# byu-magicc/VI-EKF

Hardware: AMD Instinct MI355X
Metric: EKF steps/sec (IMU-rate propagate + N_feat updates), batch=1024, N_feat=50 (higher is better)
Workload: dtype f64

## Files before the change

### vi_ekf_amd/csrc/viekf_kernels_resident.hpp

```cpp
#pragma once
#include "viekf_resident_common.hpp"
#include "viekf_resident_prop.hpp"
#include "viekf_resident_worker.hpp"
#include "viekf_resident_service.hpp"

namespace viekf {


template <int T>
__device__ __forceinline__ void res_prologue(const StreamArgs& a, ResShared& S, double* smem, int do_prop,
                                             const double* __restrict__ dt_all, const double* __restrict__ z_all,
                                             const int* __restrict__ slot_all, int M, int m_stride,
                                             const double* __restrict__ R_all, long r_stride_b, long r_stride_m,
                                             int* __restrict__ result_all) {
  const int b = blockIdx.x, tid = threadIdx.x;
  const ResLds L(a.N, a.n, a.nxs);
  S.xs = smem + L.xs; S.Kt = smem + L.Kt; S.Wt = smem + L.Wt; S.Praw = smem + L.Praw; S.lam = smem + L.lam;
  S.sm = smem + L.sm; S.fixadd = smem + L.fixadd; S.fixset = smem + L.fixset; S.Z = smem + L.Z; S.img_len = L.img_len;
  S.phiff = smem + L.phiff; S.Abb = smem + L.Abb; S.Gb = smem + L.Gb; S.Phibb = smem + L.Phibb; S.Mbb = smem + L.Mbb;
  S.Gdb = smem + L.Gdb; S.Pbb = smem + L.Pbb; S.T16 = smem + L.T16; S.xdb = smem + L.xdb; S.Pbc = smem + L.Pbc; S.PhibbT = smem + L.PhibbT; S.Pd = smem + L.Pd; S.PsiP = smem + L.PsiP; S.Pi = smem + L.Pi; S.Xi = smem + L.Xi; S.AvG = smem + L.AvG; S.Lbc = smem + L.Lbc;
  S.mz = smem + L.mz; S.mR = smem + L.mR;
  S.mslot = reinterpret_cast<int*>(smem + L.mslot);
  S.mseq = reinterpret_cast<int2*>(smem + L.mseq);
  S.ctx = reinterpret_cast<BodyCtx*>(smem + L.ctx);
  S.N = a.N; S.mcap = res_mcap(a.N); S.n = a.n; S.nf = 3 * a.N; S.len = a.len[b]; S.M = M; S.mstride = m_stride; S.do_prop = do_prop & 1; S.dbg = (do_prop >> 8) & 0xff; S.kp = (do_prop >> 16) > 0 ? (do_prop >> 16) : 1; S.B = a.B; S.b = b; S.stamps = a.ws;
  S.si = a.si(b); S.so = a.so(b);
  {
    const double* xg = a.x + S.si * a.nxs;
    for (int i = tid; i < a.nxs; i += T) S.xs[i] = (i < xZ + 5 * S.len) ? xg[i] : 0.0;
    for (int i = tid; i < a.n; i += T) S.lam[i] = a.lambda[i];
    for (int i = tid; i < 2 * a.N; i += T) { S.fixadd[i] = 0.0; S.fixset[i] = 0.0; }
    if (tid < 48) {
      const double lk = a.lambda[tid & 15], lq = a.lambda[16 + (tid >> 4)];
      S.Lbc[tid] = a.dp->use_partial_update ? (lk + lq - lq * lk) : 1.0;
    }
    if (tid == 0) { S.sm[42] = (do_prop & 1) ? dt_all[b] : 0.0; S.sm[40] = 0.0; S.sm[41] = 0.0; S.sm[44] = 0.0; S.sm[45] = 0.0; S.sm[46] = 0.0; S.sm[49] = 0.0; S.sm[50] = 0.0; S.sm[51] = 0.0; S.sm[32] = 0.0; S.sm[33] = 0.0; S.sm[52] = 0.0; S.sm[53] = 0.0; S.sm[54] = 0.0; S.sm[36] = 0.0; S.sm[37] = 0.0; }
    for (int mm_ = tid; mm_ < M; mm_ += T) {
      const int slot = slot_all[(long)b * m_stride + mm_];
      const double z0 = z_all[((long)b * m_stride + mm_) * 2], z1 = z_all[((long)b * m_stride + mm_) * 2 + 1];
      int code = 0;
      if (slot < 0) code = -1;
      else if (slot >= S.len) code = 3;
      else if (z0 != z0 || z1 != z1) code = 2;
      S.mslot[mm_] = (code == 0) ? slot : -1;
      S.mz[2 * mm_] = z0; S.mz[2 * mm_ + 1] = z1;
      const double* R = R_all + (long)b * r_stride_b + (long)mm_ * r_stride_m;
      S.mR[4 * mm_ + 0] = R[0]; S.mR[4 * mm_ + 1] = R[1]; S.mR[4 * mm_ + 2] = R[2]; S.mR[4 * mm_ + 3] = R[3];
      if (code != 0 && result_all) result_all[(long)b * m_stride + mm_] = code;
    }
  }
  RES_STAMP(S, tid == 0, 62);
  __syncthreads();
  if (a.smap_out && tid == 0) a.smap[b] = (int)S.so;
  for (int mm_ = tid; mm_ < M; mm_ += T) {
    int nx = mm_ + 1;
    while (nx < M && S.mslot[nx] < 0) nx++;
    S.mseq[mm_] = make_int2(nx, nx < M ? S.mslot[nx] : -1);
  }
  __syncthreads();
  RES_STAMP(S, tid == 0, 63);
}

template <int RB, int NW, bool MP = false, int NS = 1, bool ZU = false>
__global__ __launch_bounds__((NW + NS) * 64, (NW <= 3) ? 2 : 1) void k_step_resident(StreamArgs a, int do_prop,
                                                                const double* __restrict__ u_all,
                                                                const double* __restrict__ dt_all,
                                                                const double* __restrict__ z_all,
                                                                const int* __restrict__ slot_all, int M, int m_stride,
                                                                const double* __restrict__ R_all, long r_stride_b,
                                                                long r_stride_m, int* __restrict__ result_all) {
  extern __shared__ __attribute__((aligned(16))) double smem[];
  constexpr int T = (NW + NS) * 64, TW = NW * 64;
  const int tid = threadIdx.x;
  if ((int)blockIdx.x >= a.B) return;
  if (a.active && !a.active[blockIdx.x]) return;
#ifdef VIEKF_ABLATE
  {
    const int bits = (do_prop >> 8) & 0xff, st = (bits >> 4) & 7;
    const bool late = (bits & 128) ? ((blockIdx.x >> 8) & 1) != 0 : (blockIdx.x & 1) != 0;
    if (st && late) {
      const unsigned long long t0 = __builtin_amdgcn_s_memtime();
      while (__builtin_amdgcn_s_memtime() - t0 < (unsigned long long)st * 19200ull) __builtin_amdgcn_s_sleep(64);
    }
  }
#endif
  ResShared S;
  res_prologue<T>(a, S, smem, do_prop, dt_all, z_all, slot_all, M, m_stride, R_all, r_stride_b, r_stride_m, result_all);
  constexpr int SVC = (NW == 6 && NS == 1) ? 3 : NW;
  const int wave = tid >> 6;
  if (NS == 2) {
    if (wave == NW) res_service<T, MP, 1>(a, S, tid & 63, NW, u_all, dt_all, result_all);
    else if (wave == NW + 1) res_service<T, MP, 2>(a, S, tid & 63, NW, u_all, dt_all, result_all);
    else res_worker<RB, TW, MP, T, ZU>(a, S, tid);
  } else {
    if (wave == SVC) res_service<T, MP>(a, S, tid & 63, NW, u_all, dt_all, result_all);
    else res_worker<RB, TW, MP, T, ZU>(a, S, tid - (wave > SVC ? 64 : 0));
  }
}

}
```

### vi_ekf_amd/csrc/viekf_resident_common.hpp

```cpp
#pragma once
#include <type_traits>

#include "viekf_kernels_stream.hpp"

namespace viekf {

#ifndef RES_INLINE
#define RES_INLINE __forceinline__
#endif
constexpr int ZK = 9;
constexpr int ZS = 26;

__host__ __device__ inline int res_mcap(int N) { return N > 64 ? 80 : 64; }

struct ResLds {
  int xs, Kt, Wt, Praw, lam, sm, fixadd, fixset, Z, phiff, Abb, Gb, Phibb, Mbb, Gdb, Pbb, T16, xdb, ctx, Pbc, PhibbT, Pd, PsiP, Pi, Xi, AvG, Lbc, mslot, mseq, mz, mR, img_len, total;
  __host__ __device__ ResLds(int N, int n, int nxs) {
    const int nf = 3 * N;
    int o = 0;
    auto take = [&](int cnt) { int r = o; o += (cnt + 1) & ~1; return r; };
    xs = take(nxs);
    lam = take(n);
    sm = take(64);
    fixadd = take(2 * (N > 0 ? N : 1)); fixset = take(2 * (N > 0 ? N : 1));
    Z = take(nf * ZS > 4 * n ? nf * ZS : 4 * n);
    phiff = take(9 * (N > 0 ? N : 1));
    const int u0 = o;
    Abb = take(256); Gb = take(96); Phibb = take(256); PhibbT = take(256); Gdb = take(96); T16 = take(256);
    PsiP = take(ZK * 16); Pi = take(ZK * ZK); Xi = take(ZK * 16); AvG = take(18);
    const int uprop = o;
    o = u0;
    Kt = take(2 * n); Wt = take(2 * n);
    Praw = take(4 * n > 256 ? 4 * n : 256);
    Pd = take(4 * (N > 0 ? N : 1));
    if (uprop > o) o = uprop;
    img_len = o - Z;
    Mbb = take(256); Pbb = take(256);
    xdb = take(16);
    ctx = take((int)((sizeof(BodyCtx) + 7) / 8));
    Pbc = take(nf * 16);
    Lbc = take(48);
    const int mc = res_mcap(N);
    mslot = take(mc / 2); mseq = take(mc); mz = take(2 * mc); mR = take(4 * mc);
    total = o;
  }
};
__device__ __forceinline__ void wave_lds_sync() {
  __builtin_amdgcn_fence(__ATOMIC_RELEASE, "wavefront");
  __builtin_amdgcn_wave_barrier();
  __builtin_amdgcn_fence(__ATOMIC_ACQUIRE, "wavefront");
}
__device__ __forceinline__ int opaque(int v) { asm volatile("" : "+v"(v)); return v; }
typedef double v2f64 __attribute__((ext_vector_type(2)));
__device__ __forceinline__ double2 lds_ld2(const double* p) {
  const v2f64 v = *reinterpret_cast<const v2f64*>(p);
  return make_double2(v.x, v.y);
}
template <bool ON>
__device__ __forceinline__ void group_fence() {
  if (ON) {
    asm volatile("" ::: "memory");
    __builtin_amdgcn_sched_barrier(0);
  }
}
__device__ __forceinline__ double uniform_f64(double v) {
  const unsigned long long u = __double_as_longlong(v);
  const unsigned lo = __builtin_amdgcn_readfirstlane((unsigned)u), hi = __builtin_amdgcn_readfirstlane((unsigned)(u >> 32));
  return __longlong_as_double(((unsigned long long)hi << 32) | lo);
}

#ifdef VIEKF_STAMPS
#define RES_STAMP(S_, who, idx)                                                                  \
  do {                                                                                           \
    if ((S_).b == 0 && (who)) {                                                                  \
      __builtin_amdgcn_sched_barrier(0);                                                         \
      reinterpret_cast<unsigned long long*>((S_).stamps)[(idx)] = __builtin_amdgcn_s_memtime();  \
      __builtin_amdgcn_sched_barrier(0);                                                         \
    }                                                                                            \
  } while (0)
#else
#define RES_STAMP(S_, who, idx) do {} while (0)
#endif

#ifdef VIEKF_ISA_MARKS
#define RES_MARK(name)                          \
  do {                                          \
    __builtin_amdgcn_sched_barrier(0);          \
    asm volatile("; @@MARK " name);             \
    __builtin_amdgcn_sched_barrier(0);          \
  } while (0)
#else
#define RES_MARK(name) do {} while (0)
#endif

#ifdef VIEKF_ABLATE
#define RES_ABLATE(S_, bit) (((S_).dbg & (bit)) != 0)
#else
#define RES_ABLATE(S_, bit) false
#endif

typedef __attribute__((address_space(3))) volatile int lds_vint_t;

struct ResShared {
  double *xs, *Kt, *Wt, *Praw, *lam, *sm, *fixadd, *fixset, *Z, *phiff, *Abb, *Gb, *Phibb, *Mbb, *Gdb, *Pbb, *T16,
      *xdb, *Pbc, *PhibbT, *Pd, *PsiP, *Pi, *Xi, *AvG, *Lbc, *mz, *mR;
  int* mslot;
  int2* mseq;
  BodyCtx* ctx;
  int N, n, nf, len, M, mstride, do_prop, b, dbg, kp, B, img_len, mcap;
  long si, so;
  double* stamps;
};

__device__ __forceinline__ int res_next_valid(const ResShared& S, int from) {
  int m = from;
  while (m < S.M && S.mslot[m] < 0) m++;
  return m;
}

}
```

### vi_ekf_amd/csrc/viekf_resident_worker.hpp

```cpp
#pragma once
#include "viekf_resident_prop.hpp"

namespace viekf {


struct StoreChunk { int f0, f1, rb, h; };
__device__ __forceinline__ bool store_chunk_at(int f0, int N, int n, int img_len, StoreChunk& c) {
  if (f0 >= N) return false;
  c.f0 = f0;
  c.rb = (16 + 3 * f0) & ~1;
  c.h = ((n + 1) & ~1) - c.rb;
  c.f1 = min(N, f0 + max(1, img_len / (3 * c.h)));
  return true;
}
template <int T>
__device__ __forceinline__ void res_store_chunk(const StreamArgs& a, const ResShared& S, const StoreChunk& c, int tid) {
  const int n = S.n, ld = a.ld;
  double* P = a.P_out + S.so * n * ld;
  const double* img = S.Z;
  const int ncol = 3 * (c.f1 - c.f0), lane = tid & 63, w = tid >> 6;
  constexpr int NWV = T / 64;
  if ((n & 1) == 0) {
#pragma unroll 2
    for (int col = w; col < ncol; col += NWV) {
      const int j = 16 + 3 * c.f0 + col;
      const double* src = img + col * c.h - c.rb;
      for (int i0 = c.rb; i0 < n; i0 += 256) {
        double2 v[2];
#pragma unroll
        for (int u = 0; u < 2; u++) v[u] = lds_ld2(src + min(i0 + 2 * (lane + 64 * u), n - 2));
#pragma unroll
        for (int u = 0; u < 2; u++) {
          const int i = i0 + 2 * (lane + 64 * u);
          if (i < n && i + 1 >= j) *reinterpret_cast<double2*>(P + i + (long)j * ld) = v[u];
        }
      }
    }
  } else {
#pragma unroll 2
    for (int col = w; col < ncol; col += NWV) {
      const int j = 16 + 3 * c.f0 + col;
      const double* src = img + col * c.h - c.rb;
      for (int i = c.rb + lane; i < n; i += 64)
        if (i >= j) P[i + (long)j * ld] = src[i];
    }
  }
}

__device__ __forceinline__ void res_body_items(const ResShared& S, const double* kP, bool run, int id, int nthreads,
                                               int first, int last, int slot2, double* rawdst) {
  const double* wP = kP + 2 * S.n;
  double* Pbc = S.Pbc;
  const int j2 = ((first + id) & 7) * 2;
  double2 cw0 = {}, cw1 = {}, cl[3] = {};
  if (run) {
    cw0 = lds_ld2(wP + 2 * j2);
    cw1 = lds_ld2(wP + 2 * j2 + 2);
#pragma unroll
    for (int q = 0; q < 3; q++) cl[q] = lds_ld2(S.Lbc + 16 * q + j2);
  }
#pragma unroll 1
  for (int item = first + id; item < last; item += nthreads) {
    const int g = item >> 3;
    double2 cpv[3];
#pragma unroll
    for (int q = 0; q < 3; q++) cpv[q] = lds_ld2(Pbc + (3 * g + q) * 16 + j2);
    if (run) {
      double2 cki[3];
#pragma unroll
      for (int q = 0; q < 3; q++) cki[q] = lds_ld2(kP + 2 * (16 + 3 * g + q));
#pragma unroll
      for (int q = 0; q < 3; q++) {
        cpv[q].x = fma(-cl[q].x, fma(cki[q].y, cw0.y, cki[q].x * cw0.x), cpv[q].x);
        cpv[q].y = fma(-cl[q].y, fma(cki[q].y, cw1.y, cki[q].x * cw1.x), cpv[q].y);
        *reinterpret_cast<double2*>(Pbc + (3 * g + q) * 16 + j2) = cpv[q];
      }
    }
    if (g == slot2) {
      double* st = rawdst + 2 * j2;
      *reinterpret_cast<double2*>(st) = make_double2(cpv[0].x, cpv[1].x);
      *reinterpret_cast<double2*>(st + 2) = make_double2(cpv[0].y, cpv[1].y);
    }
  }
}
template <int RB, int TW, bool MP, int T = TW + 64, bool ZU = false>
__device__ __forceinline__ void res_worker(const StreamArgs& a, const ResShared& S, int tid) {
  const int N = S.N, n = S.n, ld = a.ld, nf = S.nf, len = S.len;
  double* P = a.P + S.si * n * ld;
  const int tid_ = tid;
  constexpr int NWV = TW / 64;
  const DevParams& prm = *a.dp;
  double* Pbc = S.Pbc;
  double* Pbb = S.Pbb;
  const int* __restrict__ resmap = a.resmap;
  auto blk = [&](int t, int ia, int& I, int& J) -> bool {
    const int e = resmap[ia * TW + t];
    I = e & 0xff;
    J = (e >> 8) & 0xff;
    return (e >> 16) != 0;
  };
  const bool own_diag = tid_ < N;

  double pb[RB][9];
  {
    const int tq = opaque(tid_);
#pragma unroll
    for (int ia = 0; ia < RB; ia++) {
      int I, J;
      blk(tq, ia, I, J);
      const bool up = I < J;
      const int br = 16 + 3 * (up ? J : I), bc = 16 + 3 * (up ? I : J);
      const double* pu = P + (br + (long)bc * ld);
#pragma unroll
      for (int s = 0; s < 3; s++)
#pragma unroll
        for (int r = 0; r < 3; r++) {
          const int rr = (I == J) ? max(r, s) : (up ? s : r), cc = (I == J) ? min(r, s) : (up ? r : s);
          pb[ia][r * 3 + s] = pu[rr + (long)cc * ld];
        }
    }
    for (int e = tid; e < nf * 16; e += TW) {
      const int k = e / nf, row = e - k * nf;
      Pbc[row * 16 + k] = P[(16 + row) + (long)k * ld];
    }
    for (int e = tid; e < 256; e += TW) {
      const int r = e & 15, c = e >> 4;
      Pbb[r * 16 + c] = P[max(r, c) + (long)min(r, c) * ld];
    }
  }

  auto sym_diag = [&]() {
    if (own_diag) { pb[0][3] = pb[0][1]; pb[0][6] = pb[0][2]; pb[0][7] = pb[0][5]; }
  };
  sym_diag();
  double Lff[9];
  {
    const double lf[3] = {a.lambda[16], a.lambda[17], a.lambda[18]};
#pragma unroll
    for (int r = 0; r < 3; r++)
#pragma unroll
      for (int s = 0; s < 3; s++) Lff[r * 3 + s] = uniform_f64(prm.use_partial_update ? (lf[s] + lf[r] - lf[r] * lf[s]) : 1.0);
  }
  const bool partial = prm.use_partial_update != 0;
  int par = 0;
  constexpr int NSV = (T - TW) / 64;
  auto fix_word = [&](int mb) -> double { return (NSV > 1) ? S.sm[40 + mb] + S.sm[36 + mb] : S.sm[40 + mb]; };
  RES_STAMP(S, tid == 0, 64);
  __syncthreads();
  RES_STAMP(S, tid == 0, 65);

  const int nkp = MP ? S.kp : 1;
  if (S.do_prop)
   for (int kp = 0; kp < nkp; kp++) {
    const int tk = MP ? opaque(tid) : tid;
    const double* Z = S.Z; double* phiff = S.phiff;
    res_prop_setup<TW>(a, S, tk);
    RES_STAMP(S, tid == 0, 66);
    __syncthreads();
    RES_STAMP(S, tid == 0, 67);

#pragma unroll
    for (int ia = 0; ia < RB; ia++) {
      const int tq = opaque(tid_);
      int I, J;
      const bool v = blk(tq, ia, I, J);
      const double* fj = phiff + 9 * J;
#pragma unroll
      for (int r = 0; r < 3; r++) {
        const double p0 = pb[ia][r * 3 + 0], p1 = pb[ia][r * 3 + 1], p2 = pb[ia][r * 3 + 2];
#pragma unroll
        for (int s = 0; s < 3; s++) pb[ia][r * 3 + s] = p0 * fj[s * 3 + 0] + p1 * fj[s * 3 + 1] + p2 * fj[s * 3 + 2];
      }
      const double* fi = phiff + 9 * I;
#pragma unroll
      for (int s = 0; s < 3; s++) {
        const double p0 = pb[ia][0 * 3 + s], p1 = pb[ia][1 * 3 + s], p2 = pb[ia][2 * 3 + s];
#pragma unroll
        for (int r = 0; r < 3; r++) pb[ia][r * 3 + s] = fi[r * 3 + 0] * p0 + fi[r * 3 + 1] * p1 + fi[r * 3 + 2] * p2;
      }
      if (v && I == J) {
        pb[ia][0] += a.Qx[16 + 3 * I + 0];
        pb[ia][4] += a.Qx[16 + 3 * I + 1];
        pb[ia][8] += a.Qx[16 + 3 * I + 2];
      }
      __builtin_amdgcn_sched_barrier(0);
      if (RB > 4) {
#pragma unroll
        for (int e = 0; e < 9; e++) asm volatile("" : "+v"(pb[ia][e]));
      }
      group_fence<(RB > 4)>();
    }
    RES_STAMP(S, tid == 0, 68);
    int zoff[RB];
    {
      const int tq = opaque(tid_);
#pragma unroll
      for (int ia = 0; ia < RB; ia++) {
        int I, J;
        blk(tq, ia, I, J);
        zoff[ia] = (3 * I * ZS) | ((3 * J * ZS) << 16);
      }
    }
    auto contract = [&](int k, auto crossed) {
      constexpr bool CROSS = decltype(crossed)::value;
#pragma unroll
      for (int ia = 0; ia < RB; ia++) {
        const double* zi = Z + (zoff[ia] & 0xffff) + 2 * k;
        const double* zj = Z + (zoff[ia] >> 16) + 2 * k;
        double2 xv[3], yv[3];
#pragma unroll
        for (int r = 0; r < 3; r++) xv[r] = lds_ld2(zi + r * ZS);
#pragma unroll
        for (int s = 0; s < 3; s++) yv[s] = lds_ld2(zj + s * ZS);
#pragma unroll
        for (int r = 0; r < 3; r++)
#pragma unroll
          for (int s = 0; s < 3; s++) {
            double acc = pb[ia][r * 3 + s];
            acc = fma(xv[r].x, CROSS ? yv[s].y : yv[s].x, acc);
            acc = fma(xv[r].y, CROSS ? yv[s].x : yv[s].y, acc);
            pb[ia][r * 3 + s] = acc;
          }
        if (ia & 1) group_fence<(RB > 4)>();
      }
    };
#pragma unroll 1
    for (int k = 0; k < ZK; k++) contract(k, std::true_type{});
#pragma unroll 1
    for (int k = ZK; k < ZK + 3; k++) contract(k, std::false_type{});
    sym_diag();
    RES_STAMP(S, tid == 0, 69);
    if (MP) res_prop_body<TW>(a, S, tk);
    par ^= 1;
    RES_STAMP(S, tid == 0, 70);
    __syncthreads();
    for (int e = tk; e < 256; e += TW) { const int r = e >> 4, c = e & 15; Pbb[e] = S.Mbb[min(r, c) * 16 + max(r, c)]; }
    if (MP && kp + 1 < nkp && own_diag && tid_ < len && fix_word(par ^ 1) != 0.0) {
      const int mb = par ^ 1, I = tid_;
      const double ad = S.fixadd[mb * N + I], st = S.fixset[mb * N + I];
      if (ad != 0.0) { pb[0][8] += ad; S.fixadd[mb * N + I] = 0.0; }
      if (st != 0.0) { pb[0][8] = prm.P0_feat[2]; S.fixset[mb * N + I] = 0.0; }
    }
   }

  int Ib[RB], Jb[RB];
  bool vb[RB];
#pragma unroll
  for (int ia = 0; ia < RB; ia++) vb[ia] = blk(tid_, ia, Ib[ia], Jb[ia]);
  const double p0rr = uniform_f64(prm.P0_feat[2]);
  auto bb_mask = [&](int r, int c) -> double { const double lr_ = S.lam[r], lc_ = S.lam[c]; return partial ? (lc_ + lr_ - lr_ * lc_) : 1.0; };
  double bbL0 = 1.0, bbL1 = 1.0;
  {
    constexpr int BBT0 = (TW >= 128) ? 128 : TW;
    const int ib0 = tid - (TW - BBT0);
    if (ib0 >= 0 && ib0 < 128) { bbL0 = bb_mask(ib0 >> 3, (ib0 & 7) * 2); bbL1 = bb_mask(ib0 >> 3, (ib0 & 7) * 2 + 1); }
  }
  auto apply_fixes = [&](int mb, double pending) {
    if (pending == 0.0) return;
    if (own_diag && tid_ < len) {
      VIEKF_COLD_BEGIN();
      const int I = tid_;
      const double ad = S.fixadd[mb * N + I], st = S.fixset[mb * N + I];
      if (ad != 0.0) { pb[0][8] += ad; S.fixadd[mb * N + I] = 0.0; }
      if (st != 0.0) { pb[0][8] = p0rr; S.fixset[mb * N + I] = 0.0; }
      VIEKF_COLD_END();
    }
  };
  auto extract_cols = [&](int slot, double* Pw) {
#pragma unroll
    for (int ia = 0; ia < RB; ia++) {
      const int I = Ib[ia], J = Jb[ia];
      const bool asrow = J == slot;
      const bool ascol = !asrow && I == slot;
      if (vb[ia] && (asrow || ascol)) {
        const int base = 16 + 3 * (asrow ? I : J);
        const double a0 = pb[ia][0], a1 = asrow ? pb[ia][1] : pb[ia][3];
        const double b0 = asrow ? pb[ia][3] : pb[ia][1], b1 = pb[ia][4];
        const double c0 = asrow ? pb[ia][6] : pb[ia][2], c1 = asrow ? pb[ia][7] : pb[ia][5];
        *reinterpret_cast<double2*>(Pw + 2 * (base + 0)) = make_double2(a0, a1);
        *reinterpret_cast<double2*>(Pw + 2 * (base + 1)) = make_double2(b0, b1);
        *reinterpret_cast<double2*>(Pw + 2 * (base + 2)) = make_double2(c0, c1);
      }
    }
  };

  int m = res_next_valid(S, 0);
  if (own_diag) {
    *reinterpret_cast<double2*>(S.Pd + 4 * tid_) = make_double2(pb[0][0], pb[0][1]);
    *reinterpret_cast<double2*>(S.Pd + 4 * tid_ + 2) = make_double2(pb[0][3], pb[0][4]);
  }
  int2 sq = S.mseq[min(m, S.mcap - 1)];
  if (m < S.M) {
    apply_fixes(par ^ 1, fix_word(par ^ 1));
    const int s0 = S.mslot[m];
    extract_cols(s0, S.Praw);
    if (sq.y >= 0) extract_cols(sq.y, S.Praw + 2 * n);
    const int e = opaque(tid);
    if (e < 16) {
      const int sf = (e < 8) ? s0 : sq.y, ijj = (e & 7) * 2;
      if (sf >= 0) {
        const double2 q0 = lds_ld2(Pbc + (3 * sf) * 16 + ijj);
        const double2 q1 = lds_ld2(Pbc + (3 * sf + 1) * 16 + ijj);
        double* d = S.Praw + ((e < 8) ? 0 : 2 * n) + 2 * ijj;
        *reinterpret_cast<double2*>(d) = make_double2(q0.x, q1.x);
        *reinterpret_cast<double2*>(d + 2) = make_double2(q0.y, q1.y);
      }
    }
  }
  RES_STAMP(S, tid == 0, 71);
  __syncthreads();
  __syncthreads();
  int it_ = 0;
  int cnt = 0;
  while (m < S.M) {
    const int mnext = sq.x;
    RES_MARK("worker.phase_top");
    const double* kP = (cnt & 1) ? S.Z : S.Kt;
    const double* wP = kP + 2 * n;
    __builtin_amdgcn_s_setprio(1);
    const double fixpending = fix_word(par ^ 1);
    const double gflag = S.sm[50 + (cnt & 1)];
    const double nanw = (NSV > 1) ? S.sm[44 + cnt % 3] + S.sm[52 + cnt % 3] : S.sm[44 + cnt % 3];
    sq = S.mseq[min(mnext, S.mcap - 1)];
    RES_STAMP(S, tid == 0 && it_ < 8, 80 + 4 * it_ + 1);
    RES_STAMP(S, (tid & 63) == 0 && it_ == 3, 192 + 4 * (tid >> 6) + 0);
    const int it = tid;
    constexpr int GB = (RB <= 4) ? RB : 2;
    RES_MARK("worker.block_sweep");
    const bool gated = gflag != 0.0;
    const bool run = !gated && nanw == 0.0 && !RES_ABLATE(S, 1);
    bool fixed = false;
#pragma unroll
    for (int g0 = 0; g0 < RB; g0 += GB) {
      double2 kI[GB][3], wJ[GB][3];
#pragma unroll
      for (int ig = 0; ig < GB; ig++) {
        const int ia = (g0 + ig < RB) ? g0 + ig : RB - 1;
#pragma unroll
        for (int r = 0; r < 3; r++) kI[ig][r] = lds_ld2(kP + 2 * (16 + 3 * Ib[ia] + r));
#pragma unroll
        for (int s = 0; s < 3; s++) wJ[ig][s] = lds_ld2(wP + 2 * (16 + 3 * Jb[ia] + s));
      }
      if (!fixed) { apply_fixes(par ^ 1, fixpending); fixed = true; }
      if (run) {
#pragma unroll
        for (int ig = 0; ig < GB; ig++) {
          if (g0 + ig >= RB) continue;
          const int ia = g0 + ig;
#pragma unroll
          for (int r = 0; r < 3; r++)
#pragma unroll
            for (int s = 0; s < 3; s++) {
              if (ZU && !(r == 2 && s == 2)) {
                pb[ia][r * 3 + s] = fma(-kI[ig][r].y, wJ[ig][s].y, fma(-kI[ig][r].x, wJ[ig][s].x, pb[ia][r * 3 + s]));
              } else {
                const double t = fma(kI[ig][r].y, wJ[ig][s].y, kI[ig][r].x * wJ[ig][s].x);
                pb[ia][r * 3 + s] = fma(-Lff[r * 3 + s], t, pb[ia][r * 3 + s]);
              }
            }
        }
      }
      group_fence<(RB > GB)>();
    }
    sym_diag();
    RES_MARK("worker.column_extraction");
    RES_STAMP(S, tid == 0 && it_ < 8, 160 + 4 * it_ + 0);
    double* rawdst = S.Praw + (cnt & 1) * 2 * n;
    if (sq.y >= 0 && !RES_ABLATE(S, 4) && !(RES_ABLATE(S, 8) && (cnt & 1))) extract_cols(sq.y, rawdst);
    __builtin_amdgcn_s_setprio(0);
    RES_STAMP(S, tid == 0 && it_ < 8, 160 + 4 * it_ + 1);
    RES_STAMP(S, (tid & 63) == 0 && it_ == 3, 192 + 4 * (tid >> 6) + 2);
    __builtin_amdgcn_sched_barrier(0);
    RES_MARK("worker.body_items");
    res_body_items(S, kP, run, (it >= 64) ? it - 64 : it + TW - 64, TW, 0, 8 * N, sq.y, rawdst);
    RES_MARK("worker.body_block");
    if (run) {
      constexpr int BBT = (TW >= 128) ? 128 : TW;
#pragma unroll
      for (int ib = it - (TW - BBT); ib >= 0 && ib < 128; ib += BBT) {
        const int br = ib >> 3, bc2 = (ib & 7) * 2;
        double2 bpv = *reinterpret_cast<double2*>(Pbb + br * 16 + bc2);
        const double2 kr = lds_ld2(kP + 2 * br), wr = lds_ld2(wP + 2 * br);
        const double2 k0 = lds_ld2(kP + 2 * bc2), w0 = lds_ld2(wP + 2 * bc2);
        const double2 k1 = lds_ld2(kP + 2 * bc2 + 2), w1 = lds_ld2(wP + 2 * bc2 + 2);
        const double L0 = (BBT == 128) ? bbL0 : bb_mask(br, bc2), L1 = (BBT == 128) ? bbL1 : bb_mask(br, bc2 + 1);
        const bool up0 = br <= bc2, up1 = br <= bc2 + 1;
        const double2 ka = up0 ? kr : k0, wa = up0 ? w0 : wr;
        const double2 kb = up1 ? kr : k1, wb = up1 ? w1 : wr;
        bpv.x = fma(-L0, fma(ka.y, wa.y, ka.x * wa.x), bpv.x);
        bpv.y = fma(-L1, fma(kb.y, wb.y, kb.x * wb.x), bpv.y);
        *reinterpret_cast<double2*>(Pbb + br * 16 + bc2) = bpv;
      }
    }
    RES_MARK("worker.phase_tail");
    par ^= 1;
    cnt++;
    RES_STAMP(S, tid == 0 && it_ < 8, 80 + 4 * it_ + 2);
    RES_STAMP(S, (tid & 63) == 0 && it_ == 3, 192 + 4 * (tid >> 6) + 1);
    __syncthreads();
    RES_STAMP(S, tid == 0 && it_ < 8, 80 + 4 * it_ + 3);
    RES_STAMP(S, (tid & 63) == 0 && it_ == 3, 192 + 4 * (tid >> 6) + 3);
    it_++;
    m = mnext;
  }
  RES_MARK("worker.loop_end");
  apply_fixes(par ^ 1, fix_word(par ^ 1));
  RES_STAMP(S, tid == 0, 72);
  __syncthreads();

  {
    P = a.P_out + S.so * n * ld;
    for (int e = opaque(tid); e < nf * 16; e += TW) {
      const int k = e / nf, row = e - k * nf;
      P[(16 + row) + (long)k * ld] = Pbc[row * 16 + k];
    }
    for (int e = opaque(tid); e < 256; e += TW) P[(e >> 4) + (long)(e & 15) * ld] = Pbb[e];
    double* img = S.Z;
    const int gtid = threadIdx.x;
    RES_STAMP(S, tid == 0, 224);
    StoreChunk sc;
    int ch = 0;
    for (int f0 = 0; store_chunk_at(f0, N, n, S.img_len, sc); f0 = sc.f1, ch++) {
      const int f1 = sc.f1;
      const int tq = opaque(tid_);
#pragma unroll
      for (int ia = 0; ia < RB; ia++) {
        int I, J;
        if (blk(tq, ia, I, J)) {
          if (I >= J && J >= f0 && J < f1) {
            double* d = img + (3 * (J - f0)) * sc.h + (16 + 3 * I - sc.rb);
#pragma unroll
            for (int s = 0; s < 3; s++)
#pragma unroll
              for (int r = 0; r < 3; r++) d[s * sc.h + r] = pb[ia][r * 3 + s];
          }
          if (I < J && I >= f0 && I < f1) {
            double* d = img + (3 * (I - f0)) * sc.h + (16 + 3 * J - sc.rb);
#pragma unroll
            for (int r = 0; r < 3; r++)
#pragma unroll
              for (int s = 0; s < 3; s++) d[r * sc.h + s] = pb[ia][r * 3 + s];
          }
        }
      }
      RES_STAMP(S, tid == 0 && ch < 3, 225 + 4 * ch);
      __syncthreads();
      RES_STAMP(S, tid == 0 && ch < 3, 226 + 4 * ch);
      res_store_chunk<T>(a, S, sc, gtid);
      RES_STAMP(S, tid == 0 && ch < 3, 227 + 4 * ch);
      __syncthreads();
      RES_STAMP(S, tid == 0 && ch < 3, 228 + 4 * ch);
    }
  }
  RES_STAMP(S, tid == 0, 73);
}


}
```

Baseline: 2.951 million.

## Overlap worker P-block loads with service-wave prologue and batch global loads

```diff
diff --git a/vi_ekf_amd/csrc/viekf_kernels_resident.hpp b/vi_ekf_amd/csrc/viekf_kernels_resident.hpp
--- a/vi_ekf_amd/csrc/viekf_kernels_resident.hpp
+++ b/vi_ekf_amd/csrc/viekf_kernels_resident.hpp
@@ -7,13 +7,13 @@
 namespace viekf {
 
 
-template <int T>
+template <int TP>
 __device__ __forceinline__ void res_prologue(const StreamArgs& a, ResShared& S, double* smem, int do_prop,
                                              const double* __restrict__ dt_all, const double* __restrict__ z_all,
                                              const int* __restrict__ slot_all, int M, int m_stride,
                                              const double* __restrict__ R_all, long r_stride_b, long r_stride_m,
-                                             int* __restrict__ result_all) {
-  const int b = blockIdx.x, tid = threadIdx.x;
+                                             int* __restrict__ result_all, int ptid) {
+  const int b = blockIdx.x;
   const ResLds L(a.N, a.n, a.nxs);
   S.xs = smem + L.xs; S.Kt = smem + L.Kt; S.Wt = smem + L.Wt; S.Praw = smem + L.Praw; S.lam = smem + L.lam;
   S.sm = smem + L.sm; S.fixadd = smem + L.fixadd; S.fixset = smem + L.fixset; S.Z = smem + L.Z; S.img_len = L.img_len;
@@ -23,19 +23,31 @@
   S.mslot = reinterpret_cast<int*>(smem + L.mslot);
   S.mseq = reinterpret_cast<int2*>(smem + L.mseq);
   S.ctx = reinterpret_cast<BodyCtx*>(smem + L.ctx);
-  S.N = a.N; S.mcap = res_mcap(a.N); S.n = a.n; S.nf = 3 * a.N; S.len = a.len[b]; S.M = M; S.mstride = m_stride; S.do_prop = do_prop & 1; S.dbg = (do_prop >> 8) & 0xff; S.kp = (do_prop >> 16) > 0 ? (do_prop >> 16) : 1; S.B = a.B; S.b = b; S.stamps = a.ws;
-  S.si = a.si(b); S.so = a.so(b);
-  {
+  S.N = a.N; S.mcap = res_mcap(a.N); S.n = a.n; S.nf = 3 * a.N; S.M = M; S.mstride = m_stride; S.do_prop = do_prop & 1; S.dbg = (do_prop >> 8) & 0xff; S.kp = (do_prop >> 16) > 0 ? (do_prop >> 16) : 1; S.B = a.B; S.b = b; S.stamps = a.ws;
+  if (ptid >= 0) {
+    const int tid = ptid;
     const double* xg = a.x + S.si * a.nxs;
-    for (int i = tid; i < a.nxs; i += T) S.xs[i] = (i < xZ + 5 * S.len) ? xg[i] : 0.0;
-    for (int i = tid; i < a.n; i += T) S.lam[i] = a.lambda[i];
-    for (int i = tid; i < 2 * a.N; i += T) { S.fixadd[i] = 0.0; S.fixset[i] = 0.0; }
+    for (int i0 = tid; i0 < a.nxs; i0 += 4 * TP) {
+      double v[4];
+#pragma unroll
+      for (int u = 0; u < 4; u++) { const int i = i0 + u * TP; v[u] = (i < xZ + 5 * S.len && i < a.nxs) ? xg[i] : 0.0; }
+#pragma unroll
+      for (int u = 0; u < 4; u++) { const int i = i0 + u * TP; if (i < a.nxs) S.xs[i] = v[u]; }
+    }
+    for (int i0 = tid; i0 < a.n; i0 += 4 * TP) {
+      double v[4];
+#pragma unroll
+      for (int u = 0; u < 4; u++) { const int i = i0 + u * TP; v[u] = (i < a.n) ? a.lambda[i] : 0.0; }
+#pragma unroll
+      for (int u = 0; u < 4; u++) { const int i = i0 + u * TP; if (i < a.n) S.lam[i] = v[u]; }
+    }
+    for (int i = tid; i < 2 * a.N; i += TP) { S.fixadd[i] = 0.0; S.fixset[i] = 0.0; }
     if (tid < 48) {
       const double lk = a.lambda[tid & 15], lq = a.lambda[16 + (tid >> 4)];
       S.Lbc[tid] = a.dp->use_partial_update ? (lk + lq - lq * lk) : 1.0;
     }
     if (tid == 0) { S.sm[42] = (do_prop & 1) ? dt_all[b] : 0.0; S.sm[40] = 0.0; S.sm[41] = 0.0; S.sm[44] = 0.0; S.sm[45] = 0.0; S.sm[46] = 0.0; S.sm[49] = 0.0; S.sm[50] = 0.0; S.sm[51] = 0.0; S.sm[32] = 0.0; S.sm[33] = 0.0; S.sm[52] = 0.0; S.sm[53] = 0.0; S.sm[54] = 0.0; S.sm[36] = 0.0; S.sm[37] = 0.0; }
-    for (int mm_ = tid; mm_ < M; mm_ += T) {
+    for (int mm_ = tid; mm_ < M; mm_ += TP) {
       const int slot = slot_all[(long)b * m_stride + mm_];
       const double z0 = z_all[((long)b * m_stride + mm_) * 2], z1 = z_all[((long)b * m_stride + mm_) * 2 + 1];
       int code = 0;
@@ -49,16 +61,15 @@
       if (code != 0 && result_all) result_all[(long)b * m_stride + mm_] = code;
     }
   }
-  RES_STAMP(S, tid == 0, 62);
+  RES_STAMP(S, threadIdx.x == 0, 62);
   __syncthreads();
-  if (a.smap_out && tid == 0) a.smap[b] = (int)S.so;
-  for (int mm_ = tid; mm_ < M; mm_ += T) {
+  RES_STAMP(S, threadIdx.x == 0, 63);
+  if (a.smap_out && ptid == 0) a.smap[b] = (int)S.so;
+  for (int mm_ = ptid; mm_ >= 0 && mm_ < M; mm_ += TP) {
     int nx = mm_ + 1;
     while (nx < M && S.mslot[nx] < 0) nx++;
     S.mseq[mm_] = make_int2(nx, nx < M ? S.mslot[nx] : -1);
   }
-  __syncthreads();
-  RES_STAMP(S, tid == 0, 63);
 }
 
 template <int RB, int NW, bool MP = false, int NS = 1, bool ZU = false>
@@ -85,16 +96,20 @@
   }
 #endif
   ResShared S;
-  res_prologue<T>(a, S, smem, do_prop, dt_all, z_all, slot_all, M, m_stride, R_all, r_stride_b, r_stride_m, result_all);
+  S.b = blockIdx.x; S.stamps = a.ws; S.dbg = (do_prop >> 8) & 0xff;
+  S.len = a.len[blockIdx.x]; S.si = a.si(blockIdx.x); S.so = a.so(blockIdx.x);
   constexpr int SVC = (NW == 6 && NS == 1) ? 3 : NW;
   const int wave = tid >> 6;
+  auto prologue = [&](int ptid) {
+    res_prologue<NS * 64>(a, S, smem, do_prop, dt_all, z_all, slot_all, M, m_stride, R_all, r_stride_b, r_stride_m, result_all, ptid);
+  };
   if (NS == 2) {
-    if (wave == NW) res_service<T, MP, 1>(a, S, tid & 63, NW, u_all, dt_all, result_all);
-    else if (wave == NW + 1) res_service<T, MP, 2>(a, S, tid & 63, NW, u_all, dt_all, result_all);
-    else res_worker<RB, TW, MP, T, ZU>(a, S, tid);
+    if (wave == NW) { prologue(tid - NW * 64); res_service<T, MP, 1>(a, S, tid & 63, NW, u_all, dt_all, result_all); }
+    else if (wave == NW + 1) { prologue(tid - NW * 64); res_service<T, MP, 2>(a, S, tid & 63, NW, u_all, dt_all, result_all); }
+    else res_worker<RB, TW, MP, T, ZU>(a, S, tid, prologue);
   } else {
-    if (wave == SVC) res_service<T, MP>(a, S, tid & 63, NW, u_all, dt_all, result_all);
-    else res_worker<RB, TW, MP, T, ZU>(a, S, tid - (wave > SVC ? 64 : 0));
+    if (wave == SVC) { prologue(tid & 63); res_service<T, MP>(a, S, tid & 63, NW, u_all, dt_all, result_all); }
+    else res_worker<RB, TW, MP, T, ZU>(a, S, tid - (wave > SVC ? 64 : 0), prologue);
   }
 }
 
diff --git a/vi_ekf_amd/csrc/viekf_resident_common.hpp b/vi_ekf_amd/csrc/viekf_resident_common.hpp
--- a/vi_ekf_amd/csrc/viekf_resident_common.hpp
+++ b/vi_ekf_amd/csrc/viekf_resident_common.hpp
@@ -94,9 +94,11 @@
 #endif
 
 #ifdef VIEKF_ABLATE
-#define RES_ABLATE(S_, bit) (((S_).dbg & (bit)) != 0)
+#define RES_ABLATE(S_, bit) (((S_).dbg & 0xf0) != 0x80 && ((S_).dbg & (bit)) != 0)
+#define RES_ABLATE_LS(S_, bit) (((S_).dbg & 0xf0) == 0x80 && ((S_).dbg & (bit)) != 0)
 #else
 #define RES_ABLATE(S_, bit) false
+#define RES_ABLATE_LS(S_, bit) false
 #endif
 
 typedef __attribute__((address_space(3))) volatile int lds_vint_t;
diff --git a/vi_ekf_amd/csrc/viekf_resident_worker.hpp b/vi_ekf_amd/csrc/viekf_resident_worker.hpp
--- a/vi_ekf_amd/csrc/viekf_resident_worker.hpp
+++ b/vi_ekf_amd/csrc/viekf_resident_worker.hpp
@@ -15,6 +15,7 @@
 }
 template <int T>
 __device__ __forceinline__ void res_store_chunk(const StreamArgs& a, const ResShared& S, const StoreChunk& c, int tid) {
+  if (RES_ABLATE_LS(S, 4)) return;
   const int n = S.n, ld = a.ld;
   double* P = a.P_out + S.so * n * ld;
   const double* img = S.Z;
@@ -83,15 +84,22 @@
     }
   }
 }
-template <int RB, int TW, bool MP, int T = TW + 64, bool ZU = false>
-__device__ __forceinline__ void res_worker(const StreamArgs& a, const ResShared& S, int tid) {
-  const int N = S.N, n = S.n, ld = a.ld, nf = S.nf, len = S.len;
-  double* P = a.P + S.si * n * ld;
+template <int TW>
+struct BodyColWalk {
+  int k, row, dk, dr, nf;
+  __device__ __forceinline__ BodyColWalk(int first, int nf_) : nf(nf_) {
+    nf = max(nf, 1);
+    k = first / nf; row = first - k * nf;
+    dk = __builtin_amdgcn_readfirstlane(TW / nf); dr = TW - dk * nf;
+  }
+  __device__ __forceinline__ void next() {
+    k += dk; row += dr;
+    if (row >= nf) { row -= nf; k++; }
+  }
+};
+template <int RB, int TW, bool MP, int T = TW + 64, bool ZU = false, class PRO>
+__device__ __forceinline__ void res_worker(const StreamArgs& a, ResShared& S, int tid, PRO&& prologue) {
   const int tid_ = tid;
-  constexpr int NWV = TW / 64;
-  const DevParams& prm = *a.dp;
-  double* Pbc = S.Pbc;
-  double* Pbb = S.Pbb;
   const int* __restrict__ resmap = a.resmap;
   auto blk = [&](int t, int ia, int& I, int& J) -> bool {
     const int e = resmap[ia * TW + t];
@@ -99,10 +107,12 @@
     J = (e >> 8) & 0xff;
     return (e >> 16) != 0;
   };
-  const bool own_diag = tid_ < N;
-
+
+  RES_STAMP(S, tid == 0, 60);
   double pb[RB][9];
   {
+    const int ld = a.ld;
+    const double* P = a.P + S.si * a.n * ld;
     const int tq = opaque(tid_);
 #pragma unroll
     for (int ia = 0; ia < RB; ia++) {
@@ -116,16 +126,48 @@
 #pragma unroll
         for (int r = 0; r < 3; r++) {
           const int rr = (I == J) ? max(r, s) : (up ? s : r), cc = (I == J) ? min(r, s) : (up ? r : s);
-          pb[ia][r * 3 + s] = pu[rr + (long)cc * ld];
+          pb[ia][r * 3 + s] = RES_ABLATE_LS(S, 1) ? 1e-3 * (r == s) : pu[rr + (long)cc * ld];
         }
     }
-    for (int e = tid; e < nf * 16; e += TW) {
-      const int k = e / nf, row = e - k * nf;
-      Pbc[row * 16 + k] = P[(16 + row) + (long)k * ld];
-    }
-    for (int e = tid; e < 256; e += TW) {
-      const int r = e & 15, c = e >> 4;
-      Pbb[r * 16 + c] = P[max(r, c) + (long)min(r, c) * ld];
+  }
+  RES_STAMP(S, tid == 0, 61);
+  prologue(-1);
+  const int N = S.N, n = S.n, ld = a.ld, nf = S.nf, len = S.len;
+  double* P = a.P + S.si * n * ld;
+  constexpr int NWV = TW / 64;
+  const DevParams& prm = *a.dp;
+  double* Pbc = S.Pbc;
+  double* Pbb = S.Pbb;
+  const bool own_diag = tid_ < N;
+  {
+    constexpr int LU = 8;
+    BodyColWalk<TW> w(tid, nf);
+    for (int e0 = tid; e0 < nf * 16; e0 += LU * TW) {
+      double v[LU];
+      int dst[LU];
+#pragma unroll
+      for (int u = 0; u < LU; u++, w.next()) {
+        const bool in = e0 + u * TW < nf * 16;
+        dst[u] = in ? w.row * 16 + w.k : -1;
+        v[u] = in ? P[(16 + w.row) + (long)w.k * ld] : 0.0;
+      }
+#pragma unroll
+      for (int u = 0; u < LU; u++)
+        if (dst[u] >= 0) Pbc[dst[u]] = v[u];
+    }
+    {
+      constexpr int BU = (256 + TW - 1) / TW;
+      double v[BU];
+#pragma unroll
+      for (int u = 0; u < BU; u++) {
+        const int e = tid + u * TW, r = e & 15, c = (e >> 4) & 15;
+        v[u] = P[max(r, c) + (long)min(r, c) * ld];
+      }
+#pragma unroll
+      for (int u = 0; u < BU; u++) {
+        const int e = tid + u * TW, r = e & 15, c = e >> 4;
+        if (e < 256) Pbb[r * 16 + c] = v[u];
+      }
     }
   }
 
@@ -410,9 +452,10 @@
 
   {
     P = a.P_out + S.so * n * ld;
-    for (int e = opaque(tid); e < nf * 16; e += TW) {
-      const int k = e / nf, row = e - k * nf;
-      P[(16 + row) + (long)k * ld] = Pbc[row * 16 + k];
+    {
+      const int e0 = opaque(tid);
+      BodyColWalk<TW> w(e0, nf);
+      for (int e = e0; e < nf * 16; e += TW, w.next()) P[(16 + w.row) + (long)w.k * ld] = Pbc[w.row * 16 + w.k];
     }
     for (int e = opaque(tid); e < 256; e += TW) P[(e >> 4) + (long)(e & 15) * ld] = Pbb[e];
     double* img = S.Z;
@@ -426,7 +469,7 @@
 #pragma unroll
       for (int ia = 0; ia < RB; ia++) {
         int I, J;
-        if (blk(tq, ia, I, J)) {
+        if (blk(tq, ia, I, J) && !RES_ABLATE_LS(S, 2)) {
           if (I >= J && J >= f0 && J < f1) {
             double* d = img + (3 * (J - f0)) * sc.h + (16 + 3 * I - sc.rb);
 #pragma unroll
```

Measured after the change: 3.001 million (median of 6 runs). 1.7% higher.
